# rbrito/deprecated-lame-mirror

Measured on AMD Instinct MI355X. Metric: encoded audio seconds/sec (x real-time) at 44.1kHz stereo CBR128, higher is better.
Workload: dtype f32

## Files before the change

### deprecated-lame-mirror_amd/csrc/lh_api.cpp

```cpp
#include <hip/hip_runtime.h>
#include <stdio.h>
#include <stdarg.h>
#include <stdlib.h>
#include <string.h>
#include <time.h>
#include <vector>
#include <mutex>
#include <thread>
#include <atomic>

#include "lamehip.h"
#include "lamehip_types.h"
#include "lh_host.h"
#include "lh_device.h"

extern "C" int lh_launch_encode(const LhConfig * cfg, const LhTables * T, const int16_t * pcm, const float *pcmf,
                                const LhStreamDesc * descs, LhStreamState * states,
                                LhFrameOut * out, uint8_t * bytes, int nstreams, void *stream);

extern "C" int lh_launch_encode_lsf(const LhConfig * cfg, const LhTables * T, const int16_t * pcm, const float *pcmf,
                                    const LhStreamDesc * descs, LhStreamState * states,
                                    LhFrameOut * out, uint8_t * bytes, int nstreams, void *stream);

extern "C" int lh_launch_encode_vbr(const LhConfig * cfg, const LhTables * T, const int16_t * pcm, const float *pcmf,
// ... 2538 lines not shown
        HIPCHK(hipMalloc((void **) &b->d_sum, (size_t) b->B * 2 * sizeof(long long)));
    if (!b->h_sum)
        HIPCHK(hipHostMalloc((void **) &b->h_sum, (size_t) b->B * 2 * sizeof(long long), 0));
    if (total > b->h_bytes_cap) {
        unsigned char *nb = nullptr;
        HIPCHK(hipHostMalloc((void **) &nb, (size_t) (total > 0 ? total : 1), 0));
        if (b->h_bytes)
            (void) hipHostFree(b->h_bytes);
        b->h_bytes = nb;
        b->h_bytes_cap = total;
    }
    if (batch_copy_streams(b) != 0)
        return LAMEHIP_ERR_DEVICE;
    HIPCHK(hipStreamWaitEvent(b->down_stream, b->ev_sum, 0));
    HIPCHK(hipMemcpyAsync(b->h_sum, b->d_sum, (size_t) b->B * 2 * sizeof(long long), hipMemcpyDeviceToHost, b->down_stream));
    if (total > 0)
        HIPCHK(hipMemcpyAsync(b->h_bytes, b->d_bytes, (size_t) total, hipMemcpyDeviceToHost, b->down_stream));
    HIPCHK(hipEventRecord(b->ev_down, b->down_stream));
    b->down_pending = 1;
    b->fetched = 1;
    return 0;
}

extern "C" long
lamehip_batch_bytes_ptr(lamehip_batch * b, int s, const unsigned char **p)
{
    LhDeviceScope const on_device(b ? b->device : -1);
    long    n;
    if (!b || s < 0 || s >= b->B || !b->encoded || !b->dev_pack || !p)
        return -1;
    if (!b->fetched && lamehip_batch_fetch(b) != 0)
        return LAMEHIP_ERR_DEVICE;
    HIPCHK(hipStreamSynchronize(b->down_stream));
    if (b->h_sum[2 * s + 1] != 0) {
        snprintf(g_err, sizeof(g_err), "device bit packer reported status %d for stream %d", (int) b->h_sum[2 * s + 1], s);
        return LAMEHIP_ERR_PAYLOAD;
    }
    n = (b->nframes[(size_t) s] == 0) ? 0 : (long) b->h_sum[2 * s];
    *p = b->h_bytes + b->bytes_off[(size_t) s];
    return n;
}

extern "C" int
lamehip_batch_set_device_packing(lamehip_batch * b, int on)
{
    if (!b)
        return -1;
    b->dev_pack = on != 0;
    return 0;
}

extern "C" long
lamehip_batch_get_bytes(lamehip_batch * b, int s, unsigned char *out, long out_size)
{
    LhDeviceScope const on_device(b ? b->device : -1);
    LhStreamState st;
    long    n;
    if (!b || s < 0 || s >= b->B || !b->encoded || !b->dev_pack)
        return -1;
    HIPCHK(hipStreamSynchronize(b->stream));
    HIPCHK(hipMemcpy(&st, b->d_state + s, sizeof(st), hipMemcpyDeviceToHost));
    if (st.status != 0) {
        snprintf(g_err, sizeof(g_err), "device bit packer reported status %d for stream %d", st.status, s);
        return LAMEHIP_ERR_PAYLOAD;
    }
    n = (long) st.em_next_header;
    if (b->nframes[(size_t) s] == 0)
        n = 0;
    if (n > out_size)
        return -1;
    if (n > 0)
        HIPCHK(hipMemcpy(out, b->d_bytes + b->bytes_off[(size_t) s], (size_t) n, hipMemcpyDeviceToHost));
    return n;
}

extern "C" long
lamehip_batch_get_bytes_tagged(lamehip_batch * b, int s, unsigned char *out, long out_size)
{
    LhVbrTag v;
    int     total, last_mode_ext = 0;
    long    k, pos = 0;
    if (!b || s < 0 || s >= b->B || !b->encoded || !b->dev_pack)
        return -1;
    total = lh_tag_init(&v, &b->cfg);
    if (b->rate_in)
        v.samplerate_in = b->rate_in;
// ... 146 lines not shown
extern "C" int
lamehip_batch_last_kernel_parts_ms(lamehip_batch * b, float *parts3)
{
    if (!b || !parts3)
        return -1;
    parts3[0] = b->part_ms[0];
    parts3[1] = b->part_ms[1];
    parts3[2] = b->part_ms[2];
    return b->last_split;
}

extern "C" int
lamehip_batch_last_windows(lamehip_batch * b)
{
    return b ? b->last_windows : 0;
}

extern "C" int
lamehip_batch_kernel_waves(lamehip_batch * b)
{
    return b ? 2 : 0;
}

extern "C" int
lamehip_batch_get_frames(lamehip_batch * b, int s, void *frames_out, int max_frames)
{
    LhDeviceScope const on_device(b ? b->device : -1);
    int     n;
    if (!b || s < 0 || s >= b->B || !b->encoded)
        return -1;
    n = b->nframes[(size_t) s];
    if (n > max_frames)
        n = max_frames;
    HIPCHK(hipStreamSynchronize(b->stream));
    HIPCHK(hipMemcpy(frames_out, b->d_out + b->out_off[(size_t) s], (size_t) n * sizeof(LhFrameOut),
                     hipMemcpyDeviceToHost));
    return n;
}


extern "C" int
lamehip_get_state(const lame_t g, void *out, int size)
{
    LhDeviceScope const on_device(valid(g) ? g->device : -1);
    if (!g || !g->have_device || size < (int) sizeof(LhStreamState))
        return -1;
    HIPCHK(hipStreamSynchronize(g->stream));
    HIPCHK(hipMemcpy(out, g->d_state, sizeof(LhStreamState), hipMemcpyDeviceToHost));
    return (int) sizeof(LhStreamState);
}

extern "C" int
lamehip_batch_get_state(lamehip_batch * b, int s, void *out, int size)
{
    LhDeviceScope const on_device(b ? b->device : -1);
    if (!b || s < 0 || s >= b->B || size < (int) sizeof(LhStreamState))
        return -1;
// ... 78 lines not shown
    lh_tag_crc(&v, out + total, k);
    if (lh_tag_frame(&v, &b->cfg, b->cfg.vbr_q, batch_padding(b, s), n > 0 ? fr[(size_t) n - 1].mode_ext : 0,
                     out, total) != total)
        memset(out, 0, (size_t) total);
    return k + total;
}

extern "C" int
lamehip_batch_pack_all(lamehip_batch * b, int nthreads, unsigned char *out, long out_stride, long *sizes)
{
    LhDeviceScope const on_device(b ? b->device : -1);
    int     dev = 0, maxf = 0;
    std::atomic < int >failed(0);
    std::mutex first_lock;
    int     first_code = 0;
    char    first_text[sizeof(g_err)] = "";
    if (!b || !b->encoded || !out || !sizes || out_stride <= 0)
        return -1;
    if (nthreads < 1)
        nthreads = 1;
    if (nthreads > b->B)
        nthreads = b->B;
    HIPCHK(hipStreamSynchronize(b->stream));
    HIPCHK(hipGetDevice(&dev));
    for (int s = 0; s < b->B; s++)
        maxf = b->nframes[(size_t) s] > maxf ? b->nframes[(size_t) s] : maxf;
    {
        std::vector < std::thread > pool;
        for (int t = 0; t < nthreads; t++)
            pool.emplace_back([=, &failed, &first_lock, &first_code, &first_text] () {
                auto note = [&](long code, const char *text) {
                    std::lock_guard < std::mutex > hold(first_lock);
                    if (first_code == 0) {
                        first_code = (int) code;
                        snprintf(first_text, sizeof(first_text), "%s", text);
                    }
                    failed = 1;
                };
                LhFrameOut *h = nullptr;
                hipStream_t st = nullptr;
                if (hipSetDevice(dev) != hipSuccess
                    || hipHostMalloc((void **) &h, (size_t) (maxf > 0 ? maxf : 1) * sizeof(LhFrameOut), 0) != hipSuccess
                    || hipStreamCreateWithFlags(&st, hipStreamNonBlocking) != hipSuccess) {
                    note(LAMEHIP_ERR_DEVICE, "pack_all: a worker could not set up its device staging");
                    for (int s = t; s < b->B; s += nthreads)
                        sizes[s] = LAMEHIP_ERR_DEVICE;
// ... 36 lines not shown
```

### deprecated-lame-mirror_amd/csrc/lh_dev_common.h

```cpp
#ifndef LH_DEV_COMMON_H
#define LH_DEV_COMMON_H

#include <stdint.h>
#include "lamehip_types.h"
#include "lh_device.h"
#include "lh_wave.h"
#include "lh_dev_math.h"

#define LH_NT 128
#ifdef LH_LSF
#define LH_NGR 1
#define LH_IS_LSF 1
#define LH_RATE8K(c) ((c).rate8k)
#else
#define LH_NGR 2
#define LH_IS_LSF 0
#define LH_RATE8K(c) 0
#endif
#define LH_BLOCK LH_NT
#define LH_SQRT2 1.41421356237309504880

#ifdef LH_EMU
#define LH_SYNC_WG() do { __syncthreads(); } while (0)
#define LH_SYNC_WG_LDS() do { __syncthreads(); } while (0)
// ... 363 lines not shown
    float   ath_adjust_factor;
    float   ath_adjust_limit;
    float   pefirbuf[19];
    int     slot_lag;
    int     ResvSize;
    int     ResvMax;
    int     main_data_begin;
    int     OldValue[2];
    int     CurrentStep[2];
    float   masking_lower;
    int     substep_shaping;
    int     frame_number;
    int     primed;
    int     status;
};
#define LH_SS_WORDS_A 50
#define LH_SS_WORDS_B 32
static_assert(sizeof(LhSmallState) == 4 * (LH_SS_WORDS_A + LH_SS_WORDS_B), "LhSmallState is two runs of words");
static_assert(__builtin_offsetof(LhStreamState, ath_adjust_limit) - __builtin_offsetof(LhStreamState, loudness_sq_save)
              == 4 * (LH_SS_WORDS_A - 1), "first run of LhStreamState's small members");
static_assert(__builtin_offsetof(LhStreamState, status) - __builtin_offsetof(LhStreamState, pefirbuf)
              == 4 * (LH_SS_WORDS_B - 1), "second run of LhStreamState's small members");

#ifdef LH_CUSTOM_LDS
#include LH_CUSTOM_LDS
#else
struct LhLds {
    LhSmallState ss;
    float   psy_en[3][4][LH_XMIN_N];
    float   psy_thm[3][4][LH_XMIN_N];
    int     psy_slot;
    float   pe[2][4];
    float   tot_ener[2][4];
    float   loudness_sq[2][2];
    float   sub_short_factor[4][3];
    int8_t  ns_attacks[4][4];
    int     ns_uselong[4];
    int     uselongblock[2];
    int     next_blocktype[2];
    int     block_type[2][2];
    int     mode_ext, padding, mean_bits, max_bits, frame_bits;
    int     targ_bits[2];
    int     bits_used[2];
    float   pe_use[2][2];
    float   ms_ener_ratio[2];
    int     scfsi[2][4];
    int     gr0_done[2];
#if defined(LH_PROF) && !defined(LH_EMU)
    unsigned prof[2][LH_NPROF];
#endif
    LhCtxShared ctx;
    LhRgSlot rg[2];
    union __attribute__((aligned(16))) {
        float   mf[2][LH_MF_NEEDED];
        struct {
            float   xr[2][2][576];
            LhQTabs qt;
            union {
                LhVbrSave vbr[2][2];
#ifdef LH_VBR_OLD
                LhVbrOldSave old[2][2];
#endif
            };
        };
    };
    union __attribute__((aligned(16))) {
// ... 329 lines not shown
```

### deprecated-lame-mirror_amd/csrc/lh_dev_qloop.h

```cpp
#ifndef LH_DEV_QLOOP_H
#define LH_DEV_QLOOP_H

#include "lh_dev_quant.h"


struct LhQS {
    float   xp[10];
    uint32_t pw[5];
    int     bnd[5];
    uint32_t vm[5];
    int     bigq;
    int     bq[5];
    float   lmax;
    int     sfw, sfbest;
    float   rxmin;
    int     wid, sta, win, pre;
    int     pnstep;
    float   pnnoise, pnlog;
    float   dist;
    int     ph;
    int     tselw, tselb;
    float   istepv, thrv;
    int     sbg8;
    int     sfbl;
// ... 1198 lines not shown
        for (int k = 0; k < 10; k++)
            keep->xpb[k] = S.xp[k];
        keep->lmaxb = S.lmax;
    }
}

template < int NS, int OLD = 0 > LH_DEVFN int
lq_outer_loop(const LhCtx & c, LhQS & S, LhChanLds & Q, LhQR & R, LhGrR & gb, const float *xr, int ch, int targ_bits,
              int sfb21_extra = 0, LhQOld * keep = nullptr)
{
    LhGrR   gw;
    LhNoiseRes best_noise_info;
    LhNoiseTmp nt;
    int     huff_bits, better, age;
    int     best_part2_3_length = 9999999;

    {
        LH_PT(t_bs);
        LQ_T(S, 40);
        (void) lq_bin_search < NS > (c, S, R, gb, Q, targ_bits, ch);
        LQ_T(S, 41);
        LH_PA(7, t_bs);
    }
    best_noise_info.over_count = 100;
    if (c.ns) {
        R.pn_global_gain = 0;
        R.pn_sfb_count1 = 0;
        if (OLD) {
            S.pnstep = 0;
            S.pnnoise = 0;
            S.pnlog = 0;
        }
        lq_noise_point < NS > (c, S, R, gb, Q, xr, nt, best_noise_info);
        best_noise_info.bits = gb.part2_3_length;
        lq_keep_best < NS, OLD > (c, S, Q, keep);
        gw = gb;
        age = 0;
        LQ_T(S, 42);
        do {
            LhNoiseRes noise_info;
            int const search_limit = (R.substep_shaping & 2) ? 20 : 3;
            int     maxggain = 255;
            if (OLD && sfb21_extra) {
                int const s = c.lane;
                int const hit = (s == R.sfbmax || (R.block_type == LH_SHORT_TYPE && (s == R.sfbmax + 1 || s == R.sfbmax + 2)))
                    && S.dist > 1.0f;
// ... 360 lines not shown
```

### deprecated-lame-mirror_amd/csrc/lh_dev_quant.h

```cpp
#ifndef LH_DEV_QUANT_H
#define LH_DEV_QUANT_H

#include "lh_dev_common.h"

#define LH_MAGIC_FLOAT (65536*(128))
#define LH_MAGIC_INT 0x4b000000

LH_DEVCONST int lh_slen1_n[16] = { 1, 1, 1, 1, 8, 2, 2, 2, 4, 4, 4, 8, 8, 8, 16, 16 };
LH_DEVCONST int lh_slen2_n[16] = { 1, 2, 4, 8, 1, 2, 4, 8, 2, 4, 8, 2, 4, 8, 4, 8 };
LH_DEVCONST int lh_slen1_tab[16] = { 0, 0, 0, 0, 3, 1, 1, 1, 2, 2, 2, 3, 3, 3, 4, 4 };
LH_DEVCONST int lh_slen2_tab[16] = { 0, 1, 2, 3, 0, 1, 2, 3, 1, 2, 3, 1, 2, 3, 2, 3 };
LH_DEVCONST int lh_scfsi_band[5] = { 0, 6, 11, 16, 21 };
LH_DEVCONST int lh_scale_short[16] = { 0, 18, 36, 54, 54, 36, 54, 72, 54, 72, 90, 72, 90, 108, 108, 126 };
LH_DEVCONST int lh_scale_long[16] = { 0, 10, 20, 30, 33, 21, 31, 41, 32, 42, 52, 43, 53, 63, 64, 74 };
LH_DEVCONST int lh_huf_tbl_noESC[15] = { 1, 2, 5, 7, 7, 10, 10, 13, 13, 13, 13, 13, 13, 13, 13 };

LH_DEVFN int
lh_ht_off(int t)
{
    switch (t) {
    case 1: return 0;
    case 2: return 4;
    case 3: return 13;
    case 5: return 22;
// ... 1617 lines not shown
    tilt = tilt > .5 ? .5 : tilt;
    shift = (int) (tilt * .5 * (targ_bits[0] + targ_bits[1]));
    if (shift > LH_MAX_BITS_PER_CHANNEL - targ_bits[0])
        shift = LH_MAX_BITS_PER_CHANNEL - targ_bits[0];
    shift = shift < 0 ? 0 : shift;
    if (targ_bits[1] >= 125) {
        int const side_after = targ_bits[1] - shift;
        if (side_after > 125) {
            targ_bits[0] += (targ_bits[0] < mean_bits) ? shift : 0;
            targ_bits[1] = side_after;
        }
        else {
            targ_bits[0] += targ_bits[1] - 125;
            targ_bits[1] = 125;
        }
    }
    both = targ_bits[0] + targ_bits[1];
    if (both > max_bits) {
        targ_bits[0] = (max_bits * targ_bits[0]) / both;
        targ_bits[1] = (max_bits * targ_bits[1]) / both;
    }
}

#endif
```

### deprecated-lame-mirror_amd/csrc/lh_device.h

```cpp
#ifndef LH_DEVICE_H
#define LH_DEVICE_H

#include "lamehip_types.h"

#ifdef __cplusplus
extern "C" {
#endif

#define LH_NPROF 44
#define LH_EMIT_HQ_MAX 256
#define LH_XMIN_N 61

enum LhRoute {
    LH_RT_S4, LH_RT_S5, LH_RT_S4n, LH_RT_S5n, LH_RT_S4m, LH_RT_S5m, LH_RT_S4s, LH_RT_S5s, LH_RT_S4t, LH_RT_S5t,
    LH_RT_O4, LH_RT_O5, LH_RT_O4n, LH_RT_O5n, LH_RT_O4m, LH_RT_O5m,
    LH_RT_OLD_PASS_FRAMES, LH_RT_OLD_PASS_EXTRA,
    LH_RT_PREP_n, LH_RT_PREP_gen, LH_RT_FIN_n, LH_RT_FIN_gen,
    LH_RT_V_n, LH_RT_V_gen, LH_RT_V_PASS2,
    LH_RT_ZERO_norm, LH_RT_ZERO_short, LH_RT_ZERO_other,
    LH_NROUTE
};

typedef struct LhStreamState {
    float   nb_l1[4][LH_CBANDS];
    float   nb_l2[4][LH_CBANDS];
    float   en[4][LH_XMIN_N + 3];
    float   thm[4][LH_XMIN_N + 3];
    float   loudness_sq_save[2];
    float   tot_ener[4];
    float   last_en_subshort[4][9];
    int     last_attacks[4];
    int     blocktype_old[2];
    float   ath_adjust_factor;
// ... 8 lines not shown
    int     CurrentStep[2];
    float   masking_lower;
    int     substep_shaping;
    int     frame_number;
    int     primed;
    int     status;
    int     pad[3];
    long long em_next_header;
    long long em_cursor;
    long long em_hq[LH_EMIT_HQ_MAX];
    int     em_nq;
    int     em_anc_flag;
    uint32_t em_part[2][2][132];
    unsigned long long prof[2][LH_NPROF];
#ifdef LH_DEBUG_DUMP
    uint32_t dbg_route[2][LH_NROUTE];
    float   dbg_xr[2][2][576];
    float   dbg_xmin[2][2][LH_SFBMAX + 1];
    float   dbg_en[2][2][LH_XMIN_N + 3];
    float   dbg_thm[2][2][LH_XMIN_N + 3];
    float   dbg_pe[2][2];
    int     dbg_targ[2][2];
    int     dbg_mean_bits;
    int     dbg_pad[3];
#endif
} LhStreamState;

typedef struct LhStreamDesc {
    long long pcm_l;
    long long pcm_r;
    long long pcm_base;
    long long nsamples;
    long long out_index;
    int     frame_begin;
    int     frame_end;
    long long bytes_base;
    long long bytes_cap;
    int     flush;
    int     mid_rel;
} LhStreamDesc;

typedef struct LhMidGr {
    float   peak[4][12];
    float   tot_ener[4];
    float   loud[2];
    float   sub_short_factor[4][3];
    int8_t  ns_attacks[4][4];
// ... 43 lines not shown
```

### deprecated-lame-mirror_amd/csrc/lh_kernels.hip

```cpp
#include <stdint.h>
#include <math.h>

#ifdef LH_EMU
#include "hipemu.h"
#define LH_CONST static const
#else
#include <hip/hip_runtime.h>
#define LH_CONST __device__ static const
#endif

#ifdef LH_EMU
#include <string.h>
#if defined(LH_LSF) || defined(LH_SPLIT)
extern "C" { extern int lh_emu_poison_lds; }
#else
extern "C" { int lh_emu_poison_lds = 0; }
#endif
#endif
#include "lh_static_tables.h"
#include "lh_dev_common.h"
#include "lh_dev_psy.h"
#include "lh_dev_mdct.h"
#include "lh_dev_quant.h"
#include "lh_dev_qloop.h"
// ... 232 lines not shown
{
    if (lh_lane() == 0)
        __hip_atomic_store(&lh_prio_tab[me], left, __ATOMIC_RELAXED, __HIP_MEMORY_SCOPE_AGENT);
    int const other = lh_uni_i(__hip_atomic_load(&lh_prio_tab[me ^ 1], __ATOMIC_RELAXED, __HIP_MEMORY_SCOPE_AGENT));
    return (left > other + LH_PRIO_BAND) ? 1 : (left + LH_PRIO_BAND < other) ? -1 : 0;
}
#define LH_PRIO_INDEX() lh_prio_index()
#define LH_PRIO_TICK(me, left) lh_prio_tick(me, left)
#define LH_PRIO_APPLY(rel, late) lh_prio_apply(rel, late)
#else
#define LH_PRIO_INDEX() 0
#define LH_PRIO_TICK(me, left) 0
#define LH_PRIO_APPLY(rel, late) do { } while (0)
#endif


#if defined(LH_BAR_LDS) && !defined(LH_EMU)
#define LH_SYNC_FRAME() LH_SYNC_WG_LDS()
#else
#define LH_SYNC_FRAME() LH_SYNC_WG()
#endif

LH_DEVFN void
lh_encode_frame(LhCtx & c, LhFrameOut * fo, LhWaveCarry & carry)
{
    LhLds & L = lh_lds;
    const LhConfig *cfg = c.cfg;
    const LhTables *T = c.T;
    LhStreamState *st = c.st;
    int const w = c.wave, lane = c.lane, tid = c.tid;
    int const nch = cfg->channels;
    constexpr int ngr = LH_NGR, fs = 576 * LH_NGR;

#if defined(LH_PROF) && !defined(LH_EMU)
    if (lane < LH_NPROF)
        L.prof[w][lane] = 0;
#endif
    LH_PT(t_frame);
#ifdef LH_SPLIT
    if (tid == 0)
        lh_lds.ss.primed = 1;
    {
        const LhMidFrame *rec = LH_AS_GLOBAL(const LhMidFrame, L.ctx.mid);
        const lh_f32x4 *sx = (const lh_f32x4 *) rec->xr.xr, *sm = (const lh_f32x4 *) &rec->small;
        lh_f32x4 *dx = (lh_f32x4 *) L.xr, *dm = (lh_f32x4 *) &L.u.psy.mid.small;
        constexpr int NM = (int) ((sizeof(LhMidSmall) + sizeof(LhMidLong)) / 16);
// ... 65 lines not shown

    float   ms_ener_ratio[2] = { .5f, .5f };
    if (cfg->mode == LH_MODE_JOINT_STEREO) {
        for (int gr = 0; gr < ngr; gr++) {
            float   r = L.tot_ener[gr][2] + L.tot_ener[gr][3];
            if (r > 0)
                r = L.tot_ener[gr][3] / r;
            ms_ener_ratio[gr] = lh_uni_f(r);
        }
    }

    {
        float   factor = lh_lds.ss.ath_adjust_factor, limit = lh_lds.ss.ath_adjust_limit;
        float   loud[2][2];
        loud[0][0] = L.loudness_sq[0][0];
        loud[1][0] = L.loudness_sq[ngr - 1][0];
        loud[0][1] = (cfg->channels == 2) ? L.loudness_sq[0][1] : loud[0][0];
        loud[1][1] = (cfg->channels == 2) ? L.loudness_sq[ngr - 1][1] : loud[1][0];
        lh_adjust_ATH(T, loud, &factor, &limit);
        LH_SYNC_FRAME();
        if (tid == 0) {
            lh_lds.ss.ath_adjust_factor = factor;
            lh_lds.ss.ath_adjust_limit = limit;
        }
    }
    LH_SYNC_FRAME();

    LH_PA(25, t_frame);
    LH_PT(t_mdct);
#ifndef LH_SPLIT
#pragma unroll
    for (int k = 0; k < 9; k++)
        L.u.mdct.sb[w][0][lane + 64 * k] = carry.sb[k];
    lh_polyphase(w);
    LH_SYNC_WG();
    lh_mdct_granules(w);
#pragma unroll
    for (int k = 0; k < 9; k++)
        carry.sb[k] = L.u.mdct.sb[w][ngr][lane + 64 * k];
    LH_SYNC_WG();
#endif
    LH_PA(2, t_mdct);
#ifndef LH_SPLIT
    lh_stage_loop_tables(c);
    LH_SYNC_WG();
#endif
// ... 103 lines not shown
        ResvMax = lh_uni_i(ResvMax);
    }
    if (abr)
        for (int gr = 0; gr < 2; gr++)
            for (int ch = 0; ch < 2; ch++)
                abr_targ[gr][ch] = lh_uni_i(abr_targ[gr][ch]);
    analog_silence_bits = lh_uni_i(analog_silence_bits);
    if (mode_ext == LH_MPG_MD_MS_LR && !vbr_new) {
        float const k = (float) (LH_SQRT2 * 0.5);
        for (int i = tid; i < ngr * 576; i += LH_NT) {
            int const gr = i >= 576, at = i - 576 * gr;
            float const l = L.xr[0][gr][at];
            float const r = L.xr[1][gr][at];
            L.xr[0][gr][at] = (l + r) * k;
            L.xr[1][gr][at] = (l - r) * k;
        }
    }
    if (ngr == 1) {
        uint32_t *z = (uint32_t *) &fo->gr[1][w];
        for (int i = lane; i < (int) (sizeof(LhGranule) / 4); i += 64)
            z[i] = 0u;
    }
    int     prepared = 0, prepared_nonzero = 0;
    for (int gr = 0; gr < ngr && !vbr_new; gr++) {
        int     targ_bits[2] = { abr_targ[gr][0], abr_targ[gr][1] };
        int     max_bits = 0;
        if (!abr)
            max_bits = lh_on_pe(cfg, ResvSize, ResvMax, &substep, pe_use[gr], targ_bits, mean_bits, gr);
        LH_SYNC_FRAME();
        substep = lh_uni_i(substep);
        if (mode_ext == LH_MPG_MD_MS_LR && !abr)
            lh_reduce_side(targ_bits, ms_ener_ratio[gr], mean_bits, max_bits);
        targ_bits[0] = lh_uni_i(targ_bits[0]);
        targ_bits[1] = lh_uni_i(targ_bits[1]);
#ifdef LH_DEBUG_DUMP
        if (tid == 0) {
            for (int ch = 0; ch < 2; ch++) {
                st->dbg_pe[gr][ch] = pe_use[gr][ch];
                st->dbg_targ[gr][ch] = targ_bits[ch];
            }
            st->dbg_mean_bits = mean_bits;
        }
#endif
        LH_SYNC_FRAME();
        if (w >= nch) {
            uint32_t *z = (uint32_t *) &fo->gr[gr][w];
            for (int i = lane; i < (int) (sizeof(LhGranule) / 4); i += 64)
                z[i] = 0u;
            if (lane == 0)
                L.bits_used[w] = 0;
        }
        else {
            int const ch = w;
            LhChanLds & Q = L.u.quant.ch[ch];
            LhQR    R;
            LhGrR   g;
            float  *xr = L.xr[ch][gr];
            LhGranule *o = &fo->gr[gr][ch];
            LH_PT(t_q);
            int const nonzero = prepared ? prepared_nonzero : lh_prepare_granule(c, ch, gr, msoff, substep);
            R = lh_uniform(L.rg[ch].R);
            g = lh_uniform(L.rg[ch].g);
            if (nonzero) {
                LH_PA(4, t_q);
                LH_PT(t_ol);
                if (abr && !R.ath_over)
                    targ_bits[ch] = analog_silence_bits;
// ... 50 lines not shown
            else
                LH_ROUTE(c, LH_ROUTE_ZERO(R.block_type));
            LH_PT(t_fin);
            lh_rg_put(c, R, g);
            if (lh_uni_i(lh_granule_is_usual(c, R.block_type, R.substep_shaping))) {
                LH_ROUTE(c, LH_RT_FIN_n);
                lh_best_scalefac_store_n(ch, gr, fo->gr[0][ch].scalefac, L.block_type[0][ch]);
                if (cfg->use_best_huffman == 1)
                    lh_best_huffman_divide_n(ch);
            }
            else {
                LH_ROUTE(c, LH_RT_FIN_gen);
                lh_best_scalefac_store(ch, gr, fo->gr[0][ch].scalefac, L.block_type[0][ch]);
                if (cfg->use_best_huffman == 1)
                    lh_best_huffman_divide(ch);
            }
            g = lh_uniform(L.rg[ch].g);
            LH_PA(6, t_fin);
            lh_store_granule(c, Q, R, g, xr, o);
            LH_DBG_XR(c, gr, ch, xr);
            if (lh_uni_i(L.ctx.bytes != nullptr))
                lh_emit_part_stage(ch, gr);
            LH_PA(3, t_q);
            if (lane == 0)
                L.bits_used[ch] = g.part2_3_length + g.part2_length;
            if (gr == 0 && nch == 2 && ngr == 2) {
                int const stamp = lh_uni_i(lh_lds.ss.frame_number) + 1;
                int     first;
                LH_WAVE_SYNC();
                first = (int) lh_bcast_u32((uint32_t) *(volatile int *) &L.gr0_done[1 - ch], 0) != stamp;
                if (lane == 0)
                    *(volatile int *) &L.gr0_done[ch] = stamp;
                carry.prio_late = !first;
                if (first) {
                    prepared_nonzero = lh_prepare_granule(c, ch, 1, msoff, substep);
                    prepared = 1;
                }
            }
            else if (nch == 2) {
                int const stamp = -(lh_uni_i(lh_lds.ss.frame_number) + 1);
                LH_WAVE_SYNC();
                carry.prio_late = (int) lh_bcast_u32((uint32_t) *(volatile int *) &L.gr0_done[1 - ch], 0) == stamp;
                if (lane == 0)
                    *(volatile int *) &L.gr0_done[ch] = stamp;
            }
        }
        LH_SYNC_FRAME();
        LH_PRIO_APPLY(carry.prio_rel, carry.prio_late);
        {
            int const used = lh_uni_i(L.bits_used[0] + L.bits_used[1]);
            ResvSize -= used;
            total_bits += used;
        }
        LH_SYNC_FRAME();
    }
    if (abr) {
        int     i, mb, rm;
        for (i = cfg->vbr_min_bitrate_index; i < cfg->vbr_max_bitrate_index; i++)
            if (lh_vbr_full_bits(cfg, i, ResvSize, &mb, &rm) >= 0)
                break;
        (void) lh_vbr_full_bits(cfg, i, ResvSize, &mb, &rm);
        bitrate_index = i;
        frame_bits = lh_frame_bits(cfg, bitrate_index, 0);
        mean_bits = mb;
        ResvMax = rm;
    }
    LH_PA(27, t_frame);
    int     drain_pre = 0, drain_post = 0;
    {
        int     stuffingBits = 0, over_bits;
        ResvSize += mean_bits * LH_NGR;
// ... 30 lines not shown
        fo->mode_ext = (int8_t) mode_ext;
        for (int i = 0; i < 7; i++)
            fo->pad[i] = 0;
        fo->resv_size = ResvSize;
        fo->frame_bits = frame_bits;
        lh_lds.ss.slot_lag = slot_lag;
        lh_lds.ss.ResvSize = ResvSize;
        lh_lds.ss.ResvMax = ResvMax;
        lh_lds.ss.main_data_begin = mdb;
        lh_lds.ss.substep_shaping = substep;
        lh_lds.ss.masking_lower = vbr_new ? masking_lower_left
            : (L.block_type[ngr - 1][nch - 1] != LH_SHORT_TYPE) ? cfg->masking_lower_long : cfg->masking_lower_short;
        lh_lds.ss.frame_number = lh_lds.ss.frame_number + 1;
        if (mdb * 8 != ResvSize)
            lh_lds.ss.status |= 1;
    }
    if (lh_uni_i(L.ctx.bytes != nullptr))
        lh_emit_frame(fo, drain_pre, drain_post, frame_bits / 8, mdb_header, bitrate_index, padding, mode_ext,
                      c.d.flush && (int) ((c.frame_base + LH_MF_START) / fs) == c.d.frame_end - 1);
    LH_PA(0, t_frame);
    LH_SYNC_FRAME();
#if defined(LH_PROF) && !defined(LH_EMU)
    if (lane < LH_NPROF)
        st->prof[w][lane] += L.prof[w][lane];
    LH_SYNC_WG();
#endif
}

#ifndef LH_WAVES_PER_EU
#define LH_WAVES_PER_EU 2
#endif
#if !defined(LH_EMU) && !defined(LH_NO_RESTRICT)
#define LH_RESTRICT __restrict__
#else
#define LH_RESTRICT
#endif
#if defined(LH_LSF) && !defined(LH_SPLIT)
#define lh_encode_kernel lh_encode_kernel_lsf
#define lh_launch_encode lh_launch_encode_lsf
#define lh_emu_encode lh_emu_encode_lsf
#define lh_emu_encode_bytes lh_emu_encode_bytes_lsf
#endif
#if defined(LH_VBRK) && !defined(LH_SPLIT)
#define lh_encode_kernel lh_encode_kernel_vbr
#define lh_launch_encode lh_launch_encode_vbr
#endif
#ifdef LH_SPLIT
// ... 292 lines not shown
}

extern "C" int
lh_launch_scatter(const int16_t * arena, int16_t * pool, long cap, const int *seg, int nseg, void *stream)
{
    if (nseg <= 0)
        return 0;
    hipLaunchKernelGGL(lh_scatter_kernel, dim3((unsigned) (2 * nseg)), dim3(256), 0, (hipStream_t) stream, arena, pool, cap,
                       seg);
    return (int) hipGetLastError();
}

#endif
#if defined(LH_TRACE) && !defined(LH_EMU)
extern "C" int
lh_trace_fetch(unsigned long long *dst)
{
    static unsigned long long zero[2][2][LH_NTRACE];
    if (hipMemcpyFromSymbol(dst, HIP_SYMBOL(lh_trace_buf), sizeof(zero)) != hipSuccess)
        return -1;
    return hipMemcpyToSymbol(HIP_SYMBOL(lh_trace_buf), zero, sizeof(zero)) == hipSuccess ? 0 : -1;
}
#endif
#ifndef LH_EMU
extern "C" int
lh_launch_encode(const LhConfig * cfg, const LhTables * T, const int16_t * pcm, const float *pcmf,
                 const LhStreamDesc * descs, LhStreamState * states, LhFrameOut * out, uint8_t * bytes,
                 int nstreams, void *stream LH_MID_PARAM)
{
    if (nstreams <= 0)
        return 0;
    hipLaunchKernelGGL(lh_encode_kernel, dim3((unsigned) nstreams), dim3(LH_BLOCK), 0,
                       (hipStream_t) stream, cfg, T, pcm, pcmf, descs, states, out, bytes, nstreams LH_MID_ARG);
    return (int) hipGetLastError();
}

#elif defined(LH_SPLIT)
extern "C" int
lh_emu_encode_q(const LhConfig * cfg, const LhTables * T, const int16_t * pcm, const float *pcmf,
                const LhStreamDesc * descs, LhStreamState * states, LhFrameOut * out, uint8_t * bytes, int nstreams,
                const LhMidPools * pools)
{
    hipemu_dim3 grid = { (unsigned) nstreams, 1, 1 }, block = { LH_BLOCK, 1, 1 };
    LhMidPools const mid = *pools;
    hipemu_run(grid, block,[=] () {
               lh_encode_kernel(cfg, T, pcm, pcmf, descs, states, out, bytes, nstreams, mid);
// ... 35 lines not shown
```

### deprecated-lame-mirror_amd/csrc/lh_wave.h

```cpp
#ifndef LH_WAVE_H
#define LH_WAVE_H

#include <stdint.h>

#define LH_RARE(x) __builtin_expect(!!(x), 0)
#define LH_OFTEN(x) __builtin_expect(!!(x), 1)

#ifdef LH_EMU
#include "hipemu.h"

static inline int lh_lane(void) { return hipemu_lane(); }
static inline int lh_wave_id(void) { return hipemu_wave(); }
#define LH_WAVE_SYNC() hipemu_wave_sync()
#define LH_WAVE_SYNC_MEM() hipemu_wave_sync()
#define LH_WAVE_ORDER() hipemu_wave_sync()
#define LH_SCHED_FENCE() do { } while (0)

static inline uint32_t
lh_wave_sum_u32(uint32_t v)
{
    const uint64_t *x = hipemu_wave_exchange(v);
    uint32_t s = 0;
    for (int i = 0; i < 64; i++)
        s += (uint32_t) x[i];
// ... 219 lines not shown
        uint32_t s = 0;
        int const g = hipemu_lane() & ~7;
        for (int k = 0; k < 8; k++)
            s += (uint32_t) x[g + k];
        v[i] = s;
    }
}

template < int N > static inline void
lh_wave_sum_tail3(uint32_t (&v)[N])
{
    for (int i = 0; i < N; i++) {
        const uint64_t *x = hipemu_wave_exchange(v[i]);
        uint32_t s = 0;
        for (int k = 0; k < 64; k += 8)
            s += (uint32_t) x[k];
        v[i] = s;
    }
}

static inline void lh_lds_add(int *p, int v) { *p += v; }
static inline void lh_lds_max(int *p, int v) { if (v > *p) *p = v; }
static inline void lh_lds_addf(float *p, float v) { *p += v; }
static inline int lh_uni_i(int v) { return v; }
static inline uint32_t lh_vec_u32(uint32_t v) { return v; }
static inline float lh_uni_f(float v) { return v; }
static inline long long lh_uni_ll(long long v) { return v; }
static inline double lh_uni_f64(double v) { return v; }
static inline int lh_ffs64(uint64_t m) { return m ? __builtin_ctzll(m) : -1; }
static inline int lh_popc64(uint64_t m) { return __builtin_popcountll(m); }
static inline int lh_clz64(uint64_t m) { return m ? __builtin_clzll(m) : 64; }
static inline int lh_clz32(uint32_t m) { return m ? __builtin_clz(m) : 32; }
static inline double lh_fma(double a, double b, double c) { return __builtin_fma(a, b, c); }

#else
#include <hip/hip_runtime.h>

__device__ __forceinline__ int lh_lane(void) { return (int) (threadIdx.x & 63); }
__device__ __forceinline__ int lh_wave_id(void) { return (int) (threadIdx.x >> 6); }

#define LH_WAVE_SYNC() do { __builtin_amdgcn_fence(__ATOMIC_ACQ_REL, "workgroup", "local"); \
                            __builtin_amdgcn_wave_barrier(); } while (0)
#define LH_WAVE_ORDER() do { asm volatile("" ::: "memory"); __builtin_amdgcn_wave_barrier(); \
                             asm volatile("" ::: "memory"); } while (0)
#define LH_SCHED_FENCE() __builtin_amdgcn_sched_barrier(0)
#define LH_WAVE_SYNC_MEM() LH_WAVE_SYNC()
// ... 237 lines not shown

__device__ __forceinline__ uint32_t
lh_lds_off(const void *p)
{
    return (uint32_t) (uintptr_t) (const __attribute__((address_space(3))) char *) p;
}

__device__ __forceinline__ uint32_t
lh_lds_read_u32(uint32_t off)
{
    return *(const __attribute__((address_space(3))) uint32_t *) (uintptr_t) off;
}

__device__ __forceinline__ uint32_t
lh_dot2_u16(uint32_t a, uint32_t b, uint32_t c)
{
    typedef unsigned short lh_u16x2_ __attribute__((ext_vector_type(2)));
    return __builtin_amdgcn_udot2(__builtin_bit_cast(lh_u16x2_, a), __builtin_bit_cast(lh_u16x2_, b), c, false);
}

__device__ __forceinline__ void lh_lds_add(int *p, int v) { (void) __hip_atomic_fetch_add(p, v, __ATOMIC_RELAXED, __HIP_MEMORY_SCOPE_WORKGROUP); }
__device__ __forceinline__ void lh_lds_max(int *p, int v) { (void) __hip_atomic_fetch_max(p, v, __ATOMIC_RELAXED, __HIP_MEMORY_SCOPE_WORKGROUP); }
__device__ __forceinline__ void lh_lds_addf(float *p, float v) { (void) __hip_atomic_fetch_add(p, v, __ATOMIC_RELAXED, __HIP_MEMORY_SCOPE_WORKGROUP); }

__device__ __forceinline__ int lh_uni_i(int v) { return __builtin_amdgcn_readfirstlane(v); }
__device__ __forceinline__ uint32_t lh_vec_u32(uint32_t v) { asm volatile("" : "+v"(v)); return v; }
__device__ __forceinline__ float lh_uni_f(float v) { return __int_as_float(__builtin_amdgcn_readfirstlane(__float_as_int(v))); }
__device__ __forceinline__ long long lh_uni_ll(long long v)
{
    unsigned const lo = (unsigned) __builtin_amdgcn_readfirstlane((int) (unsigned) (unsigned long long) v);
    unsigned const hi = (unsigned) __builtin_amdgcn_readfirstlane((int) (unsigned) ((unsigned long long) v >> 32));
    return (long long) (((unsigned long long) hi << 32) | lo);
}
__device__ __forceinline__ double lh_uni_f64(double v) { return __longlong_as_double(lh_uni_ll(__double_as_longlong(v))); }
__device__ __forceinline__ int lh_ffs64(uint64_t m) { return m ? (__ffsll((long long) m) - 1) : -1; }
__device__ __forceinline__ int lh_popc64(uint64_t m) { return __popcll(m); }
__device__ __forceinline__ int lh_clz64(uint64_t m) { return __clzll((long long) m); }
__device__ __forceinline__ int lh_clz32(uint32_t m) { return __clz((int) m); }
__device__ __forceinline__ double lh_fma(double a, double b, double c) { return __fma_rn(a, b, c); }

#endif

#endif
```

Before: 84250.

## Decouple granule-1 start from granule-0 barrier when the bit budget is provably fixed

Each channel wave publishes a bound on its granule-0 bit usage. After finishing granule 0, a wave checks whether granule 1's target bits are identical across every reservoir level the other channel could leave. If so, it skips the frame-wide barrier and goes straight to granule 1, with an LDS compare-and-swap picking the decision so both waves agree. This removes idle time where one channel waits on the other between granules, at the cost of extra bound bookkeeping, a new status bit for bound violations, and a host-side status check before packing.

```diff
diff --git a/deprecated-lame-mirror_amd/csrc/lh_api.cpp b/deprecated-lame-mirror_amd/csrc/lh_api.cpp
--- a/deprecated-lame-mirror_amd/csrc/lh_api.cpp
+++ b/deprecated-lame-mirror_amd/csrc/lh_api.cpp
@@ -2584,6 +2584,8 @@
     return 0;
 }
 
+static void status_text(int status, int s);
+
 extern "C" long
 lamehip_batch_bytes_ptr(lamehip_batch * b, int s, const unsigned char **p)
 {
@@ -2595,7 +2597,7 @@
         return LAMEHIP_ERR_DEVICE;
     HIPCHK(hipStreamSynchronize(b->down_stream));
     if (b->h_sum[2 * s + 1] != 0) {
-        snprintf(g_err, sizeof(g_err), "device bit packer reported status %d for stream %d", (int) b->h_sum[2 * s + 1], s);
+        status_text((int) b->h_sum[2 * s + 1], s);
         return LAMEHIP_ERR_PAYLOAD;
     }
     n = (b->nframes[(size_t) s] == 0) ? 0 : (long) b->h_sum[2 * s];
@@ -2623,7 +2625,7 @@
     HIPCHK(hipStreamSynchronize(b->stream));
     HIPCHK(hipMemcpy(&st, b->d_state + s, sizeof(st), hipMemcpyDeviceToHost));
     if (st.status != 0) {
-        snprintf(g_err, sizeof(g_err), "device bit packer reported status %d for stream %d", st.status, s);
+        status_text(st.status, s);
         return LAMEHIP_ERR_PAYLOAD;
     }
     n = (long) st.em_next_header;
@@ -2816,6 +2818,33 @@
     return b ? 2 : 0;
 }
 
+static void
+status_text(int status, int s)
+{
+    if (status & LH_STATUS_BOUND)
+        snprintf(g_err, sizeof(g_err), "device reported status %d for stream %d (bit %d: a channel spent more bits on granule 0 "
+                 "than the bound the other channel relied on for granule 1's budget)", status, s, LH_STATUS_BOUND);
+    else
+        snprintf(g_err, sizeof(g_err), "device bit packer reported status %d for stream %d", status, s);
+}
+
+static int
+batch_bound_ok(lamehip_batch * b, int s0, int n)
+{
+    std::vector < int >st((size_t) (n > 0 ? n : 1));
+    if (n <= 0)
+        return 1;
+    if (hipMemcpy2D(st.data(), sizeof(int), (const char *) (b->d_state + s0) + offsetof(LhStreamState, status),
+                    sizeof(LhStreamState), sizeof(int), (size_t) n, hipMemcpyDeviceToHost) != hipSuccess)
+        return -1;
+    for (int i = 0; i < n; i++)
+        if (st[(size_t) i] & LH_STATUS_BOUND) {
+            status_text(st[(size_t) i], s0 + i);
+            return 0;
+        }
+    return 1;
+}
+
 extern "C" int
 lamehip_batch_get_frames(lamehip_batch * b, int s, void *frames_out, int max_frames)
 {
@@ -2827,6 +2856,11 @@
     if (n > max_frames)
         n = max_frames;
     HIPCHK(hipStreamSynchronize(b->stream));
+    {
+        int const ok = batch_bound_ok(b, s, 1);
+        if (ok <= 0)
+            return ok < 0 ? LAMEHIP_ERR_DEVICE : LAMEHIP_ERR_PAYLOAD;
+    }
     HIPCHK(hipMemcpy(frames_out, b->d_out + b->out_off[(size_t) s], (size_t) n * sizeof(LhFrameOut),
                      hipMemcpyDeviceToHost));
     return n;
@@ -2951,6 +2985,11 @@
     if (nthreads > b->B)
         nthreads = b->B;
     HIPCHK(hipStreamSynchronize(b->stream));
+    {
+        int const ok = batch_bound_ok(b, 0, b->B);
+        if (ok <= 0)
+            return ok < 0 ? LAMEHIP_ERR_DEVICE : LAMEHIP_ERR_PAYLOAD;
+    }
     HIPCHK(hipGetDevice(&dev));
     for (int s = 0; s < b->B; s++)
         maxf = b->nframes[(size_t) s] > maxf ? b->nframes[(size_t) s] : maxf;
diff --git a/deprecated-lame-mirror_amd/csrc/lh_dev_common.h b/deprecated-lame-mirror_amd/csrc/lh_dev_common.h
--- a/deprecated-lame-mirror_amd/csrc/lh_dev_common.h
+++ b/deprecated-lame-mirror_amd/csrc/lh_dev_common.h
@@ -409,6 +409,11 @@
 static_assert(__builtin_offsetof(LhStreamState, status) - __builtin_offsetof(LhStreamState, pefirbuf)
               == 4 * (LH_SS_WORDS_B - 1), "second run of LhStreamState's small members");
 
+#define LH_DECIDE_GO 1
+#define LH_DECIDE_WAIT 2
+#define LH_BOUND_NONE (-1)
+#define LH_BOUND_FINAL 0x4000
+
 #ifdef LH_CUSTOM_LDS
 #include LH_CUSTOM_LDS
 #else
@@ -426,9 +431,11 @@
     int     uselongblock[2];
     int     next_blocktype[2];
     int     block_type[2][2];
-    int     mode_ext, padding, mean_bits, max_bits, frame_bits;
+    int     mean_bits, max_bits, frame_bits;
     int     targ_bits[2];
     int     bits_used[2];
+    int     gr_decide;
+    short   gr_bound[2];
     float   pe_use[2][2];
     float   ms_ener_ratio[2];
     int     scfsi[2][4];
diff --git a/deprecated-lame-mirror_amd/csrc/lh_dev_qloop.h b/deprecated-lame-mirror_amd/csrc/lh_dev_qloop.h
--- a/deprecated-lame-mirror_amd/csrc/lh_dev_qloop.h
+++ b/deprecated-lame-mirror_amd/csrc/lh_dev_qloop.h
@@ -1244,6 +1244,12 @@
         LQ_T(S, 41);
         LH_PA(7, t_bs);
     }
+    if (!OLD && c.lane == 0) {
+        int const now = gb.part2_3_length + gb.part2_length;
+        int const had = *(volatile short *) &lh_lds.gr_bound[ch];
+        if (had == LH_BOUND_NONE || !(had & LH_BOUND_FINAL))
+            *(volatile short *) &lh_lds.gr_bound[ch] = (short) (now > targ_bits ? now : targ_bits);
+    }
     best_noise_info.over_count = 100;
     if (c.ns) {
         R.pn_global_gain = 0;
diff --git a/deprecated-lame-mirror_amd/csrc/lh_dev_quant.h b/deprecated-lame-mirror_amd/csrc/lh_dev_quant.h
--- a/deprecated-lame-mirror_amd/csrc/lh_dev_quant.h
+++ b/deprecated-lame-mirror_amd/csrc/lh_dev_quant.h
@@ -1663,4 +1663,33 @@
     }
 }
 
+LH_DEVFN int
+lh_budget_is_fixed(const LhConfig * cfg, int ResvSize_lo, int ResvSize_hi, int ResvMax, int substep, const float pe[2],
+                   int mean_bits, int mode_ext, float ms_ener_ratio, int targ_bits_out[2])
+{
+    if (cfg->vbr == 3)
+        return 1;
+    if (ResvSize_lo > ResvSize_hi)
+        return 0;
+    {
+        int const usable = (substep & 1) ? (int) (ResvMax * 0.9) : ResvMax;
+        if ((ResvSize_hi + mean_bits) * 10 > usable * 9)
+            return 0;
+    }
+    int     f_lo = substep, f_hi = substep, t_lo[2], t_hi[2];
+    int const max_lo = lh_on_pe(cfg, ResvSize_lo, ResvMax, &f_lo, pe, t_lo, mean_bits, 1);
+    int const max_hi = lh_on_pe(cfg, ResvSize_hi, ResvMax, &f_hi, pe, t_hi, mean_bits, 1);
+    if (max_hi >= LH_MAX_BITS_PER_GRANULE || t_lo[0] != t_hi[0] || t_lo[1] != t_hi[1] || ((f_lo ^ f_hi) & 0x80))
+        return 0;
+    if (mode_ext == LH_MPG_MD_MS_LR) {
+        lh_reduce_side(t_lo, ms_ener_ratio, mean_bits, max_lo);
+        lh_reduce_side(t_hi, ms_ener_ratio, mean_bits, max_hi);
+        if (t_lo[0] != t_hi[0] || t_lo[1] != t_hi[1])
+            return 0;
+    }
+    targ_bits_out[0] = t_hi[0];
+    targ_bits_out[1] = t_hi[1];
+    return 1;
+}
+
 #endif
diff --git a/deprecated-lame-mirror_amd/csrc/lh_device.h b/deprecated-lame-mirror_amd/csrc/lh_device.h
--- a/deprecated-lame-mirror_amd/csrc/lh_device.h
+++ b/deprecated-lame-mirror_amd/csrc/lh_device.h
@@ -9,6 +9,7 @@
 
 #define LH_NPROF 44
 #define LH_EMIT_HQ_MAX 256
+#define LH_STATUS_BOUND 64
 #define LH_XMIN_N 61
 
 enum LhRoute {
@@ -63,7 +64,8 @@
     float   dbg_pe[2][2];
     int     dbg_targ[2][2];
     int     dbg_mean_bits;
-    int     dbg_pad[3];
+    uint32_t dbg_decouple[2];
+    int     dbg_pad[1];
 #endif
 } LhStreamState;
 
diff --git a/deprecated-lame-mirror_amd/csrc/lh_kernels.hip b/deprecated-lame-mirror_amd/csrc/lh_kernels.hip
--- a/deprecated-lame-mirror_amd/csrc/lh_kernels.hip
+++ b/deprecated-lame-mirror_amd/csrc/lh_kernels.hip
@@ -278,6 +278,59 @@
 #endif
 
 LH_DEVFN void
+lh_gr1_targets(const LhConfig * cfg, int level, int ResvMax, int substep, const float pe[2], int mean_bits, int mode_ext,
+               float ms_ener_ratio, int t[2])
+{
+    if (cfg->vbr != 3) {
+        int const max_bits = lh_on_pe(cfg, level, ResvMax, &substep, pe, t, mean_bits, 1);
+        if (mode_ext == LH_MPG_MD_MS_LR)
+            lh_reduce_side(t, ms_ener_ratio, mean_bits, max_bits);
+    }
+}
+
+#ifdef LH_EMU
+#define LH_DECIDE_FENCE() do { } while (0)
+#else
+#define LH_DECIDE_FENCE() __builtin_amdgcn_fence(__ATOMIC_SEQ_CST, "workgroup")
+#endif
+
+#if defined(LH_EMU)
+extern "C" { extern unsigned lh_emu_decouple[2]; }
+#define LH_DECOUPLE_COUNT(decider, go) do { if ((decider) && lane == 0) { lh_emu_decouple[0] += 1u; lh_emu_decouple[1] += (go) ? 1u : 0u; } } while (0)
+#elif defined(LH_DEBUG_DUMP)
+#define LH_DECOUPLE_COUNT(decider, go) do { if ((decider) && lane == 0) { \
+        __hip_atomic_fetch_add(&st->dbg_decouple[0], 1u, __ATOMIC_RELAXED, __HIP_MEMORY_SCOPE_AGENT); \
+        __hip_atomic_fetch_add(&st->dbg_decouple[1], (go) ? 1u : 0u, __ATOMIC_RELAXED, __HIP_MEMORY_SCOPE_AGENT); } } while (0)
+#else
+#define LH_DECOUPLE_COUNT(decider, go) do { } while (0)
+#endif
+#if defined(LH_PROF) && !defined(LH_EMU) && defined(LH_SPLIT)
+#define LH_SKEW_AT(gr, wv) (*(volatile unsigned *) &L.prof[1][(gr) ? ((wv) ? 38 : 37) : ((wv) ? 28 : 12)])
+#define LH_SKEW_PROVEN (*(volatile unsigned *) &L.prof[1][39])
+#define LH_SKEW_SCRATCH(wv, slot) ((wv) == 1 && ((slot) == 12 || (slot) == 28 || ((slot) >= 37 && (slot) <= 39)))
+#define LH_SKEW_WOULD(x) do { if ((x) && lane == 0) { L.prof[w][14] += 1u; LH_SKEW_PROVEN = 1u; } } while (0)
+#define LH_SKEW_ARRIVE(gr) do { if (lane == 0 && w < 2) LH_SKEW_AT(gr, w) = (unsigned) clock64(); } while (0)
+#define LH_SKEW_LEAVE(gr, both) do { if (lane == 0 && w < 2) { \
+        L.prof[w][(gr) ? 16 : 17] += (unsigned) clock64() - LH_SKEW_AT(gr, w); \
+        if ((gr) == 1 && w == 0 && (both)) { \
+            int const d0 = (int) (LH_SKEW_AT(0, 1) - LH_SKEW_AT(0, 0)), d1 = (int) (LH_SKEW_AT(1, 1) - LH_SKEW_AT(1, 0)); \
+            int const a0 = d0 < 0 ? -d0 : d0, a1 = d1 < 0 ? -d1 : d1, ds = d0 + d1 < 0 ? -(d0 + d1) : d0 + d1; \
+            L.prof[0][15] += 1u; \
+            L.prof[0][12] += (unsigned) a0; \
+            L.prof[0][28] += (unsigned) a1; \
+            L.prof[0][39] += ((d0 < 0) == (d1 < 0)) ? 1u : 0u; \
+            L.prof[0][37] += (unsigned) ((a0 + a1 - ds) / 2); \
+            if (LH_SKEW_PROVEN) \
+                L.prof[0][38] += (unsigned) ((a0 + a1 - ds) / 2); \
+        } } } while (0)
+#else
+#define LH_SKEW_WOULD(x) do { } while (0)
+#define LH_SKEW_ARRIVE(gr) do { } while (0)
+#define LH_SKEW_LEAVE(gr, both) do { } while (0)
+#define LH_SKEW_SCRATCH(wv, slot) 0
+#endif
+
+LH_DEVFN void
 lh_encode_frame(LhCtx & c, LhFrameOut * fo, LhWaveCarry & carry)
 {
     LhLds & L = lh_lds;
@@ -389,6 +442,8 @@
         if (tid == 0) {
             lh_lds.ss.ath_adjust_factor = factor;
             lh_lds.ss.ath_adjust_limit = limit;
+            L.gr_decide = 0;
+            L.gr_bound[0] = L.gr_bound[1] = LH_BOUND_NONE;
         }
     }
     LH_SYNC_FRAME();
@@ -538,15 +593,23 @@
             z[i] = 0u;
     }
     int     prepared = 0, prepared_nonzero = 0;
+    int const pair = (ngr == 2 && nch == 2 && !vbr_new);
+    int     go = 0, go1[2] = { 0, 0 };
     for (int gr = 0; gr < ngr && !vbr_new; gr++) {
         int     targ_bits[2] = { abr_targ[gr][0], abr_targ[gr][1] };
         int     max_bits = 0;
-        if (!abr)
-            max_bits = lh_on_pe(cfg, ResvSize, ResvMax, &substep, pe_use[gr], targ_bits, mean_bits, gr);
-        LH_SYNC_FRAME();
-        substep = lh_uni_i(substep);
-        if (mode_ext == LH_MPG_MD_MS_LR && !abr)
-            lh_reduce_side(targ_bits, ms_ener_ratio[gr], mean_bits, max_bits);
+        if (gr == 1 && go) {
+            targ_bits[0] = go1[0];
+            targ_bits[1] = go1[1];
+        }
+        else {
+            if (!abr)
+                max_bits = lh_on_pe(cfg, ResvSize, ResvMax, &substep, pe_use[gr], targ_bits, mean_bits, gr);
+            LH_SYNC_FRAME();
+            substep = lh_uni_i(substep);
+            if (mode_ext == LH_MPG_MD_MS_LR && !abr)
+                lh_reduce_side(targ_bits, ms_ener_ratio[gr], mean_bits, max_bits);
+        }
         targ_bits[0] = lh_uni_i(targ_bits[0]);
         targ_bits[1] = lh_uni_i(targ_bits[1]);
 #ifdef LH_DEBUG_DUMP
@@ -558,7 +621,8 @@
             st->dbg_mean_bits = mean_bits;
         }
 #endif
-        LH_SYNC_FRAME();
+        if (!(gr == 1 && go))
+            LH_SYNC_FRAME();
         if (w >= nch) {
             uint32_t *z = (uint32_t *) &fo->gr[gr][w];
             for (int i = lane; i < (int) (sizeof(LhGranule) / 4); i += 64)
@@ -655,8 +719,16 @@
             if (lh_uni_i(L.ctx.bytes != nullptr))
                 lh_emit_part_stage(ch, gr);
             LH_PA(3, t_q);
-            if (lane == 0)
-                L.bits_used[ch] = g.part2_3_length + g.part2_length;
+            int const used = g.part2_3_length + g.part2_length;
+            if (lane == 0) {
+                L.bits_used[ch] = used;
+                if (gr == 0) {
+                    int const bound = *(volatile short *) &L.gr_bound[ch];
+                    if (bound != LH_BOUND_NONE && used > bound)
+                        lh_lds_or((uint32_t *) &lh_lds.ss.status, (uint32_t) LH_STATUS_BOUND);
+                    *(volatile short *) &L.gr_bound[ch] = (short) (used | LH_BOUND_FINAL);
+                }
+            }
             if (gr == 0 && nch == 2 && ngr == 2) {
                 int const stamp = lh_uni_i(lh_lds.ss.frame_number) + 1;
                 int     first;
@@ -669,6 +741,48 @@
                     prepared_nonzero = lh_prepare_granule(c, ch, 1, msoff, substep);
                     prepared = 1;
                 }
+                int     mine = LH_DECIDE_WAIT, t1[2] = { abr_targ[1][0], abr_targ[1][1] };
+                int const level = ResvSize - used;
+                LH_WAVE_SYNC();
+                int const other = (int) lh_bcast_u32((uint32_t) *(volatile short *) &L.gr_bound[1 - ch], 0);
+                if (other != LH_BOUND_NONE) {
+                    int const most = other & ~LH_BOUND_FINAL;
+                    if (other & LH_BOUND_FINAL)
+                        mine = LH_DECIDE_GO;
+                    else if (lh_budget_is_fixed(cfg, level - most, level, ResvMax, substep, pe_use[1], mean_bits, mode_ext,
+                                                ms_ener_ratio[1], t1))
+                        mine = LH_DECIDE_GO;
+                }
+                int const would = (mine == LH_DECIDE_GO);
+#ifdef LH_NO_DECOUPLE
+                mine = LH_DECIDE_WAIT;
+#endif
+#ifdef LH_EMU
+                if (lane == 0 && getenv("LH_TEST_FORCE_FIRST") && atoi(getenv("LH_TEST_FORCE_FIRST")) != ch)
+                    while (*(volatile int *) &L.gr_decide == 0)
+                        hipemu_yield();
+#endif
+                LH_DECIDE_FENCE();
+                int     seen = 0;
+                if (lane == 0)
+                    seen = lh_lds_cas(&L.gr_decide, 0, mine);
+                seen = (int) lh_bcast_u32((uint32_t) seen, 0);
+                LH_DECIDE_FENCE();
+                go = lh_uni_i((seen ? seen : mine) == LH_DECIDE_GO);
+                if (go) {
+                    if (seen || (other != LH_BOUND_NONE && (other & LH_BOUND_FINAL))) {
+                        int const its = lh_uni_i(*(volatile short *) &L.gr_bound[1 - ch]) & ~LH_BOUND_FINAL;
+                        lh_gr1_targets(cfg, level - its, ResvMax, substep, pe_use[1], mean_bits, mode_ext, ms_ener_ratio[1], t1);
+                    }
+                    go1[0] = lh_uni_i(t1[0]);
+                    go1[1] = lh_uni_i(t1[1]);
+                    if (!prepared) {
+                        prepared_nonzero = lh_prepare_granule(c, ch, 1, msoff, substep);
+                        prepared = 1;
+                    }
+                }
+                LH_DECOUPLE_COUNT(seen == 0, go);
+                LH_SKEW_WOULD(seen == 0 && would);
             }
             else if (nch == 2) {
                 int const stamp = -(lh_uni_i(lh_lds.ss.frame_number) + 1);
@@ -678,8 +792,22 @@
                     *(volatile int *) &L.gr0_done[ch] = stamp;
             }
         }
+        if (gr == 0 && go) {
+            LH_PRIO_APPLY(carry.prio_rel, carry.prio_late);
+            continue;
+        }
+        LH_SKEW_ARRIVE(gr);
         LH_SYNC_FRAME();
+        LH_SKEW_LEAVE(gr, pair && !go);
         LH_PRIO_APPLY(carry.prio_rel, carry.prio_late);
+        if (gr == 1 && go) {
+            int const used0 = lh_uni_i((L.gr_bound[0] & ~LH_BOUND_FINAL) + (L.gr_bound[1] & ~LH_BOUND_FINAL));
+            ResvSize -= used0;
+            total_bits += used0;
+            if (!abr)
+                (void) lh_granule_budget(cfg, ResvSize, ResvMax, &substep, mean_bits, 1);
+            substep = lh_uni_i(substep);
+        }
         {
             int const used = lh_uni_i(L.bits_used[0] + L.bits_used[1]);
             ResvSize -= used;
@@ -756,7 +884,7 @@
     LH_SYNC_FRAME();
 #if defined(LH_PROF) && !defined(LH_EMU)
     if (lane < LH_NPROF)
-        st->prof[w][lane] += L.prof[w][lane];
+        st->prof[w][lane] += LH_SKEW_SCRATCH(w, lane) ? 0u : L.prof[w][lane];
     LH_SYNC_WG();
 #endif
 }
@@ -1095,6 +1223,52 @@
     return hipMemcpyToSymbol(HIP_SYMBOL(lh_trace_buf), zero, sizeof(zero)) == hipSuccess ? 0 : -1;
 }
 #endif
+#if defined(LH_EMU) && !defined(LH_LSF) && !defined(LH_SPLIT)
+extern "C" {
+unsigned lh_emu_decouple[2];
+
+int
+lh_emu_budget_probe(const LhConfig * cfg, int lo, int hi, int ResvMax, int substep, float pe0, float pe1, int mean_bits,
+                    int mode_ext, float ms_ener_ratio, int *same, int *agree, int *regime)
+{
+    float const pe[2] = { pe0, pe1 };
+    int     out[2] = { -1, -1 }, first[2] = { 0, 0 }, flag0 = 0;
+    int const fixed = lh_budget_is_fixed(cfg, lo, hi, ResvMax, substep, pe, mean_bits, mode_ext, ms_ener_ratio, out);
+    *same = 1;
+    for (int level = lo; level <= hi; level++) {
+        int     t[2], f = substep;
+        int const max_bits = lh_on_pe(cfg, level, ResvMax, &f, pe, t, mean_bits, 1);
+        if (mode_ext == LH_MPG_MD_MS_LR)
+            lh_reduce_side(t, ms_ener_ratio, mean_bits, max_bits);
+        if (level == lo) {
+            first[0] = t[0];
+            first[1] = t[1];
+            flag0 = f & 0x80;
+        }
+        else if (t[0] != first[0] || t[1] != first[1] || (f & 0x80) != flag0)
+            *same = 0;
+    }
+    *agree = (out[0] == first[0] && out[1] == first[1]);
+    {
+        int     f = substep, share, most, wanted = 0;
+        LhGranuleBudget const b = lh_granule_budget(cfg, lo, ResvMax, &f, mean_bits, 1);
+        share = (LH_MAX_BITS_PER_CHANNEL < b.target / cfg->channels) ? LH_MAX_BITS_PER_CHANNEL : b.target / cfg->channels;
+        most = mean_bits * 3 / 4;
+        for (int ch = 0; ch < cfg->channels; ch++) {
+            int     w = (int) (share * pe[ch] / 700.0 - share);
+            w = w > most ? most : w;
+            w = w < 0 ? 0 : w;
+            if (w + share > LH_MAX_BITS_PER_CHANNEL)
+                w = (LH_MAX_BITS_PER_CHANNEL - share > 0) ? LH_MAX_BITS_PER_CHANNEL - share : 0;
+            wanted += w;
+        }
+        regime[0] = wanted;
+        regime[1] = b.reserve;
+    }
+    return fixed;
+}
+}
+#endif
 #ifndef LH_EMU
 extern "C" int
 lh_launch_encode(const LhConfig * cfg, const LhTables * T, const int16_t * pcm, const float *pcmf,
diff --git a/deprecated-lame-mirror_amd/csrc/lh_wave.h b/deprecated-lame-mirror_amd/csrc/lh_wave.h
--- a/deprecated-lame-mirror_amd/csrc/lh_wave.h
+++ b/deprecated-lame-mirror_amd/csrc/lh_wave.h
@@ -265,6 +265,7 @@
 static inline void lh_lds_add(int *p, int v) { *p += v; }
 static inline void lh_lds_max(int *p, int v) { if (v > *p) *p = v; }
 static inline void lh_lds_addf(float *p, float v) { *p += v; }
+static inline int lh_lds_cas(int *p, int expect, int v) { int const old = *p; if (old == expect) *p = v; return old; }
 static inline int lh_uni_i(int v) { return v; }
 static inline uint32_t lh_vec_u32(uint32_t v) { return v; }
 static inline float lh_uni_f(float v) { return v; }
@@ -548,6 +549,12 @@
 __device__ __forceinline__ void lh_lds_add(int *p, int v) { (void) __hip_atomic_fetch_add(p, v, __ATOMIC_RELAXED, __HIP_MEMORY_SCOPE_WORKGROUP); }
 __device__ __forceinline__ void lh_lds_max(int *p, int v) { (void) __hip_atomic_fetch_max(p, v, __ATOMIC_RELAXED, __HIP_MEMORY_SCOPE_WORKGROUP); }
 __device__ __forceinline__ void lh_lds_addf(float *p, float v) { (void) __hip_atomic_fetch_add(p, v, __ATOMIC_RELAXED, __HIP_MEMORY_SCOPE_WORKGROUP); }
+__device__ __forceinline__ int
+lh_lds_cas(int *p, int expect, int v)
+{
+    (void) __hip_atomic_compare_exchange_strong(p, &expect, v, __ATOMIC_RELAXED, __ATOMIC_RELAXED, __HIP_MEMORY_SCOPE_WORKGROUP);
+    return expect;
+}
 
 __device__ __forceinline__ int lh_uni_i(int v) { return __builtin_amdgcn_readfirstlane(v); }
 __device__ __forceinline__ uint32_t lh_vec_u32(uint32_t v) { asm volatile("" : "+v"(v)); return v; }
```

Measured after the change: 84180. Within noise of the previous version (-0.1%).
